# JeroendenBoef/GraphPOPE

Measured on AMD Instinct MI355X. Metric: POPE embeddings/sec (nodes x anchors) + SAGE nodes/sec, Flickr 256 anchors, higher is better.
Workload: dtype u64; 1 GPU; configs[1]: flickr-shaped geodesic-stochastic, N=89250 E=899756 F=500, 256 anchors PER GPU (np.random seed 42); inputs resident in HBM (edge_index, x) -> [N, F+K] f32 in HBM on every rank; anchors_total=256, anchors_per_rank=256, parallelism=single GPU

## Files before the change

### graphpope_amd/csrc/geodesic_level.h

```cpp
#pragma once

#ifdef POPE_STAMP
__device__ unsigned long long g_stamps[16384 * 8];
__device__ int g_stamp_level;
#define STAMP(slot)                                                                         \
    do {                                                                                    \
        __builtin_amdgcn_sched_barrier(0);                                                  \
        if (lane == 0 && wave < 16384 && level == g_stamp_level) g_stamps[wave * 8 + (slot)] = __builtin_amdgcn_s_memrealtime(); \
        __builtin_amdgcn_sched_barrier(0);                                                  \
    } while (0)
#else
#define STAMP(slot) do { } while (0)
#endif

template <int WT> struct Words { u64 w[WT]; };

typedef float f32x4 __attribute__((ext_vector_type(4)));

constexpr int DPP_ROW_SHR1 = 0x111, DPP_ROW_SHR2 = 0x112, DPP_ROW_SHR4 = 0x114, DPP_ROW_SHR8 = 0x118, DPP_ROW_BCAST15 = 0x142,
              DPP_ROW_BCAST31 = 0x143, DPP_WAVE_SHL1 = 0x130, DPP_WAVE_SHR1 = 0x138;
template <int CTRL>
__device__ __forceinline__ int dpp_mov(int x) { return __builtin_amdgcn_update_dpp(0, x, CTRL, 0xf, 0xf, true); }
template <int CTRL>
__device__ __forceinline__ u64 dpp_mov64(u64 x) {
    const unsigned lo = (unsigned)dpp_mov<CTRL>((int)(unsigned)x), hi = (unsigned)dpp_mov<CTRL>((int)(unsigned)(x >> 32));
    return ((u64)hi << 32) | lo;
}

template <int WT>
__device__ __forceinline__ Words<WT> load_words(const u64 *__restrict__ p) {
    Words<WT> r;
    if constexpr (WT == 1) {
        r.w[0] = p[0];
    } else {
#pragma unroll
        for (int i = 0; i < WT; i += 2) {
            const ulonglong2 v = *reinterpret_cast<const ulonglong2 *>(p + i);
            r.w[i] = v.x;
            r.w[i + 1] = v.y;
        }
    }
    return r;
}

typedef unsigned long long u64x2v __attribute__((ext_vector_type(2)));
typedef int i32x4v __attribute__((ext_vector_type(4)));
template <int WT, bool NT>
__device__ __forceinline__ Words<WT> load_words_hint(const u64 *__restrict__ p) {
    if constexpr (!NT) return load_words<WT>(p);
    Words<WT> r;
    if constexpr (WT == 1) {
        r.w[0] = __builtin_nontemporal_load(p);
    } else {
#pragma unroll
        for (int i = 0; i < WT; i += 2) {
            const u64x2v v = __builtin_nontemporal_load(reinterpret_cast<const u64x2v *>(p + i));
            r.w[i] = v.x;
            r.w[i + 1] = v.y;
        }
    }
    return r;
}

template <int WT>
__device__ __forceinline__ Words<WT> gather_words(const u64 *__restrict__ p) { return load_words<WT>(p); }

template <int WT>
__device__ __forceinline__ void store_words(u64 *__restrict__ p, const Words<WT> &r) {
    if constexpr (WT == 1) {
        p[0] = r.w[0];
    } else {
#pragma unroll
        for (int i = 0; i < WT; i += 2) *reinterpret_cast<ulonglong2 *>(p + i) = make_ulonglong2(r.w[i], r.w[i + 1]);
    }
}

template <int WT, bool NT>
__device__ __forceinline__ void store_words_hint(u64 *__restrict__ p, const Words<WT> &r) {
    if constexpr (!NT) {
        store_words<WT>(p, r);
    } else if constexpr (WT == 1) {
        __builtin_nontemporal_store(r.w[0], p);
    } else {
#pragma unroll
        for (int i = 0; i < WT; i += 2) {
            const u64x2v v = {r.w[i], r.w[i + 1]};
            __builtin_nontemporal_store(v, reinterpret_cast<u64x2v *>(p + i));
        }
    }
}

template <int WT>
__device__ __forceinline__ u64 any_bits(const Words<WT> &r) {
    u64 a = 0;
#pragma unroll
    for (int i = 0; i < WT; ++i) a |= r.w[i];
    return a;
}

template <int WT, bool NT = false>
__device__ __forceinline__ void commit_words(const Words<WT> &fresh, const Words<WT> &seen_old, size_t idx,
                                             u64 *__restrict__ seen, u64 *__restrict__ hop_planes,
                                             size_t plane_elems, int level) {
    Words<WT> s;
#pragma unroll
    for (int i = 0; i < WT; ++i) s.w[i] = seen_old.w[i] | fresh.w[i];
    store_words_hint<WT, NT>(seen + idx, s);
    Words<WT> h[5];
#pragma unroll
    for (int b = 0; b < 5; ++b) {
        h[b] = fresh;
        if ((level >> b) & 1) h[b] = load_words_hint<WT, NT>(hop_planes + (size_t)b * plane_elems + idx);
    }
#pragma unroll
    for (int b = 0; b < 5; ++b)
        if ((level >> b) & 1) {
#pragma unroll
            for (int i = 0; i < WT; ++i) h[b].w[i] |= fresh.w[i];
            store_words_hint<WT, NT>(hop_planes + (size_t)b * plane_elems + idx, h[b]);
        }
    for (int b = 5, l = level >> 5; l; ++b, l >>= 1)
        if (l & 1) {
            u64 *p = hop_planes + (size_t)b * plane_elems + idx;
            Words<WT> g = load_words_hint<WT, NT>(p);
#pragma unroll
            for (int i = 0; i < WT; ++i) g.w[i] |= fresh.w[i];
            store_words_hint<WT, NT>(p, g);
        }
}

__device__ __forceinline__ void stage_live_table(const unsigned *__restrict__ live, int live_words, uint4 *live_lds4) {
    const uint4 *src = reinterpret_cast<const uint4 *>(live);
    const int n4 = (live_words + 3) / 4;
    for (int base = 0; base < n4; base += 4 * 256) {
        uint4 t[4];
        int idx[4];
#pragma unroll
        for (int j = 0; j < 4; ++j) idx[j] = min(base + (int)threadIdx.x + 256 * j, n4 - 1);
#pragma unroll
        for (int j = 0; j < 4; ++j) t[j] = src[idx[j]];
#pragma unroll
        for (int j = 0; j < 4; ++j) live_lds4[idx[j]] = t[j];
    }
}

__global__ __launch_bounds__(256) void k_live_summary(const unsigned *__restrict__ live, int padded_words, unsigned *__restrict__ sum) {
    const int w = blockIdx.x * blockDim.x + threadIdx.x;
    const unsigned v = w < padded_words ? live[w] : 0u;
    const unsigned long long b = __ballot(v != 0u);
    if ((threadIdx.x & 63) == 0 && w < padded_words) {
        sum[(w >> 5)] = (unsigned)b;
        sum[(w >> 5) + 1] = (unsigned)(b >> 32);
    }
}

template <int WT, int LIVE, int TILES>
__device__ __forceinline__ void level_housekeeping(int E, int N, int Wp, int tiles_arg, const u64 *__restrict__ front, u64 *__restrict__ seen,
                                                   u64 *__restrict__ idle, u64 *__restrict__ hop_planes, size_t plane_elems, int level,
                                                   const int *aux, const unsigned *__restrict__ live, unsigned *__restrict__ live_idle,
                                                   int live_words, int t0, int tstride) {
    const int tiles = TILES ? tiles_arg : 1;
    const int n = (E + CHUNK - 1) >> CHUNK_SHIFT;
    const int *mrows = aux + AUX_HEADER;
    for (int i = t0; i < live_words; i += tstride) live_idle[i] = 0u;
    Words<WT> zero;
#pragma unroll
    for (int i = 0; i < WT; ++i) zero.w[i] = 0;
    for (int i = t0; i < n; i += tstride) {
        const int mv = mrows[i];
        if (mv >= 0)
            for (int t = 0; t < tiles; ++t) store_words<WT>(idle + (size_t)mv * Wp + t * WT, zero);
    }
    if (level > 1) {
        for (int v = t0; v < N; v += tstride) {
            if (!((live[v >> 5] >> (v & 31)) & 1u)) continue;
            constexpr bool NT = LIVE >= 2 && POPE_NT_PLANES != 0;
            for (int t = 0; t < tiles; ++t) {
                const size_t idx = (size_t)v * Wp + t * WT;
                const Words<WT> fresh = load_words<WT>(front + idx);
                if (any_bits<WT>(fresh))
                    commit_words<WT, NT>(fresh, load_words_hint<WT, NT>(seen + idx), idx, seen, hop_planes, plane_elems, level - 1);
            }
        }
    }
}

__device__ __forceinline__ int2 chunk_edge_rows(const int *__restrict__ erow, int chunk, int E) {
    int2 r = make_int2(-1, -2);
    if (chunk > 0 && chunk * CHUNK - 1 < E) r.x = erow[chunk * CHUNK - 1];
    if ((chunk + 1) * CHUNK < E) r.y = erow[(chunk + 1) * CHUNK];
    return r;
}

template <int WT, int LIVE, int TILES>
__device__ __forceinline__ bool level_expand(const int *__restrict__ erow, const int *__restrict__ col, int E, int Wp, int tile_begin, int tile_end,
                                             const u64 *__restrict__ front, u64 *__restrict__ seen, u64 *__restrict__ acc,
                                             const unsigned *__restrict__ live, unsigned *__restrict__ live_acc,
                                             const unsigned *live_lds, int level, int lane, int wave, int nwaves, int nchunks,
                                             int4 vr, int4 ur, unsigned *wave_words) {
    auto load_idx = [&](const int *p) {
        if constexpr (LIVE >= 2 && POPE_NT_INDEX != 0) {
            const i32x4v t = __builtin_nontemporal_load(reinterpret_cast<const i32x4v *>(p));
            return make_int4(t.x, t.y, t.z, t.w);
        } else {
            return *reinterpret_cast<const int4 *>(p);
        }
    };
    constexpr bool LOOP = TILES == 1;
    constexpr int TILE_AHEAD = LOOP ? (WT == 8 ? POPE_WT8_PREFETCH : POPE_TILE_PREFETCH) : 0;
    if (!TILES) { tile_begin = 0; tile_end = 1; }
    bool found = false;
    STAMP(0);
    auto live4 = [&](int u0, int u1, int u2, int u3, bool &q0, bool &q1, bool &q2, bool &q3) {
        if constexpr (LIVE == 3) {
            const bool s0 = (live_lds[u0 >> 10] >> ((u0 >> 5) & 31)) & 1u, s1 = (live_lds[u1 >> 10] >> ((u1 >> 5) & 31)) & 1u,
                       s2 = (live_lds[u2 >> 10] >> ((u2 >> 5) & 31)) & 1u, s3 = (live_lds[u3 >> 10] >> ((u3 >> 5) & 31)) & 1u;
            const unsigned w0 = live[s0 ? u0 >> 5 : 0], w1 = live[s1 ? u1 >> 5 : 0], w2 = live[s2 ? u2 >> 5 : 0], w3 = live[s3 ? u3 >> 5 : 0];
            q0 = s0 & ((w0 >> (u0 & 31)) & 1u); q1 = s1 & ((w1 >> (u1 & 31)) & 1u);
            q2 = s2 & ((w2 >> (u2 & 31)) & 1u); q3 = s3 & ((w3 >> (u3 & 31)) & 1u);
        } else {
            const unsigned *t = LIVE == 1 ? live_lds : live;
            const unsigned w0 = t[u0 >> 5], w1 = t[u1 >> 5], w2 = t[u2 >> 5], w3 = t[u3 >> 5];
            q0 = (w0 >> (u0 & 31)) & 1u; q1 = (w1 >> (u1 & 31)) & 1u; q2 = (w2 >> (u2 & 31)) & 1u; q3 = (w3 >> (u3 & 31)) & 1u;
        }
    };
    constexpr bool AHEAD = (LIVE >= 2 || (WT == 8 && POPE_L2_LOOP != 0)) && POPE_AHEAD != 0;
    constexpr bool AHEAD_LIVE = AHEAD && POPE_AHEAD == 1;
    auto slots_of = [&](int chunk, const int4 &vr_, const int4 &ur_, int &v0, int &v1, int &v2, int &v3, int &u0, int &u1, int &u2, int &u3) {
        const int base = chunk * CHUNK + lane * SLOTS;
        v0 = v1 = v2 = v3 = -1;
        u0 = u1 = u2 = u3 = 0;
        if (base < E) {
            v0 = vr_.x; u0 = ur_.x;
            if (base + 1 < E) { v1 = vr_.y; u1 = ur_.y; }
            if (base + 2 < E) { v2 = vr_.z; u2 = ur_.z; }
            if (base + 3 < E) { v3 = vr_.w; u3 = ur_.w; }
        }
    };
    bool q0 = false, q1 = false, q2 = false, q3 = false;
    if (AHEAD_LIVE && wave < nchunks) {
        int a0, a1, a2, a3, b0, b1, b2, b3;
        slots_of(wave, vr, ur, a0, a1, a2, a3, b0, b1, b2, b3);
        live4(b0, b1, b2, b3, q0, q1, q2, q3);
    }
    for (int chunk = wave; chunk < nchunks; chunk += nwaves) {
        STAMP(7);
        if (!AHEAD && chunk != wave && chunk * CHUNK + lane * SLOTS < E) {
            vr = load_idx(erow + chunk * CHUNK + lane * SLOTS);
            ur = load_idx(col + chunk * CHUNK + lane * SLOTS);
        }
        int v0, v1, v2, v3, u0, u1, u2, u3;
        slots_of(chunk, vr, ur, v0, v1, v2, v3, u0, u1, u2, u3);
        int4 vr_n = make_int4(-1, -1, -1, -1), ur_n = make_int4(0, 0, 0, 0);
        bool qn0 = false, qn1 = false, qn2 = false, qn3 = false;
        const int chunk_n = chunk + nwaves;
        if (AHEAD && chunk_n < nchunks && chunk_n * CHUNK + lane * SLOTS < E) {
            vr_n = load_idx(erow + chunk_n * CHUNK + lane * SLOTS);
            ur_n = load_idx(col + chunk_n * CHUNK + lane * SLOTS);
        }
        auto next_live = [&]() {
            if constexpr (AHEAD_LIVE) {
                if (chunk_n < nchunks) {
                    int a0, a1, a2, a3, b0, b1, b2, b3;
                    slots_of(chunk_n, vr_n, ur_n, a0, a1, a2, a3, b0, b1, b2, b3);
                    live4(b0, b1, b2, b3, qn0, qn1, qn2, qn3);
                }
            }
        };
        auto advance = [&]() {
            if constexpr (AHEAD) { vr = vr_n; ur = ur_n; }
            if constexpr (AHEAD_LIVE) { q0 = qn0; q1 = qn1; q2 = qn2; q3 = qn3; }
        };
        if constexpr (!AHEAD_LIVE) live4(u0, u1, u2, u3, q0, q1, q2, q3);
        const bool g0 = (v0 >= 0) & q0, g1 = (v1 >= 0) & q1, g2 = (v2 >= 0) & q2, g3 = (v3 >= 0) & q3;
        const int vc = __builtin_amdgcn_readlane(v0, 0);
        const int vl = __builtin_amdgcn_readlane(v3, 63);
        STAMP(1);
        const bool work = __any(g0 || g1 || g2 || g3);
        if (!work) {
            next_live();
            advance();
            continue;
        }
        const int2 er = chunk_edge_rows(erow, __builtin_amdgcn_readfirstlane(chunk), E);
        const bool head_multi = chunk > 0 && er.x == vc;
        const bool tail_multi = vl >= 0 && (chunk + 1) * CHUNK < E && er.y == vl;
        const bool x0 = (head_multi && v0 == vc) || (tail_multi && v0 == vl);
        const bool x1 = (head_multi && v1 == vc) || (tail_multi && v1 == vl);
        const bool x2 = (head_multi && v2 == vc) || (tail_multi && v2 == vl);
        const bool x3 = (head_multi && v3 == vc) || (tail_multi && v3 == vl);
        const int nv0 = dpp_mov<DPP_WAVE_SHL1>(v0);
        const int after3 = lane == 63 ? -3 : nv0;
        const bool e0 = v0 >= 0 && v0 != v1, e1 = v1 >= 0 && v1 != v2, e2 = v2 >= 0 && v2 != v3, e3 = v3 >= 0 && v3 != after3;
        const int pv3 = dpp_mov<DPP_WAVE_SHR1>(v3);
        const bool connects = lane > 0 && pv3 == v0 && v0 >= 0;
        const bool head0 = !(connects && v0 == v3);
        bool lv0, lv1, lv2, lv3;
        live4(max(v0, 0), max(v1, 0), max(v2, 0), max(v3, 0), lv0, lv1, lv2, lv3);
        bool m0 = false, m1 = false, m2 = false, m3 = false;
        const bool dense = TILES != 0;

        auto gather4 = [&](int woff, Words<WT> &c0, Words<WT> &c1, Words<WT> &c2, Words<WT> &c3) {
#pragma unroll
            for (int i = 0; i < WT; ++i) c0.w[i] = c1.w[i] = c2.w[i] = c3.w[i] = 0;
            if (g0) c0 = gather_words<WT>(front + (size_t)u0 * Wp + woff);
            if (g1) c1 = gather_words<WT>(front + (size_t)u1 * Wp + woff);
            if (g2) c2 = gather_words<WT>(front + (size_t)u2 * Wp + woff);
            if (g3) c3 = gather_words<WT>(front + (size_t)u3 * Wp + woff);
        };
        Words<WT> c0, c1, c2, c3, d0, d1, d2, d3;
        gather4(tile_begin * WT, c0, c1, c2, c3);
        if (TILE_AHEAD == 2 && tile_begin + 1 < tile_end) gather4((tile_begin + 1) * WT, d0, d1, d2, d3);
        next_live();
        for (int tile = tile_begin; tile < tile_end; ++tile) {
            const int woff = tile * WT;
            {
                auto row_mask = [&](int v, bool lv) {
                    Words<WT> m = load_words_hint<WT, LIVE >= 2 && POPE_NT_PLANES != 0>(seen + (size_t)v * Wp + woff);
                    if (lv) {
                        const Words<WT> f = load_words<WT>(front + (size_t)v * Wp + woff);
#pragma unroll
                        for (int i = 0; i < WT; ++i) m.w[i] |= f.w[i];
                    }
                    return m;
                };
                Words<WT> s0, s1, s2, s3;
#pragma unroll
                for (int i = 0; i < WT; ++i) s0.w[i] = s1.w[i] = s2.w[i] = s3.w[i] = 0;
                if (v0 >= 0) s0 = row_mask(v0, lv0);
                if (v3 >= 0) s3 = v3 == v0 ? s0 : row_mask(v3, lv3);
                if (v1 >= 0) s1 = v1 == v0 ? s0 : (v1 == v3 ? s3 : row_mask(v1, lv1));
                if (v2 >= 0) s2 = v2 == v1 ? s1 : (v2 == v3 ? s3 : row_mask(v2, lv2));
#pragma unroll
                for (int i = 0; i < WT; ++i) {
                    c0.w[i] &= ~s0.w[i];
                    c1.w[i] &= ~s1.w[i];
                    c2.w[i] &= ~s2.w[i];
                    c3.w[i] &= ~s3.w[i];
                }
            }
            if (TILE_AHEAD == 1 && tile + 1 < tile_end) gather4(woff + WT, d0, d1, d2, d3);
            const u64 any = any_bits<WT>(c0) | any_bits<WT>(c1) | any_bits<WT>(c2) | any_bits<WT>(c3);
            if (tile == tile_begin) STAMP(2);
            if (__any(any != 0)) {
#pragma unroll
                for (int i = 0; i < WT; ++i) {
                    if (v1 == v0) c1.w[i] |= c0.w[i];
                    if (v2 == v1) c2.w[i] |= c1.w[i];
                    if (v3 == v2) c3.w[i] |= c2.w[i];
                }
                Words<WT> t = c3;
                bool head = head0;
                auto scan_step = [&](auto ctrl, bool valid) {
                    constexpr int CTRL = decltype(ctrl)::value;
                    if (!__any(valid && !head)) return;
                    const bool ph = dpp_mov<CTRL>((int)head) != 0;
                    const bool take = valid && !head;
#pragma unroll
                    for (int i = 0; i < WT; ++i) {
                        const u64 pt = dpp_mov64<CTRL>(t.w[i]);
                        if (take) t.w[i] |= pt;
                    }
                    if (take) head = ph;
                };
                const int in_row = lane & 15;
                scan_step(std::integral_constant<int, DPP_ROW_SHR1>{}, in_row >= 1);
                scan_step(std::integral_constant<int, DPP_ROW_SHR2>{}, in_row >= 2);
                scan_step(std::integral_constant<int, DPP_ROW_SHR4>{}, in_row >= 4);
                scan_step(std::integral_constant<int, DPP_ROW_SHR8>{}, in_row >= 8);
                scan_step(std::integral_constant<int, DPP_ROW_BCAST15>{}, ((lane >> 4) & 1) != 0);
                scan_step(std::integral_constant<int, DPP_ROW_BCAST31>{}, lane >= 32);
#pragma unroll
                for (int i = 0; i < WT; ++i) {
                    u64 ci = dpp_mov64<DPP_WAVE_SHR1>(t.w[i]);
                    if (!connects) ci = 0;
                    c0.w[i] |= ci;
                    if (v1 == v0) c1.w[i] |= ci;
                    if (v2 == v0) c2.w[i] |= ci;
                    if (v3 == v0) c3.w[i] |= ci;
                }
            }
            if (tile == tile_begin) STAMP(3);
            const size_t i0 = (size_t)v0 * Wp + woff, i1 = (size_t)v1 * Wp + woff, i2 = (size_t)v2 * Wp + woff,
                         i3 = (size_t)v3 * Wp + woff;
            const bool n0 = e0 && any_bits<WT>(c0) != 0, n1 = e1 && any_bits<WT>(c1) != 0, n2 = e2 && any_bits<WT>(c2) != 0,
                       n3 = e3 && any_bits<WT>(c3) != 0;
            if (e0 && !x0 && (n0 || dense)) store_words<WT>(acc + i0, c0);
            if (e1 && !x1 && (n1 || dense)) store_words<WT>(acc + i1, c1);
            if (e2 && !x2 && (n2 || dense)) store_words<WT>(acc + i2, c2);
            if (e3 && !x3 && (n3 || dense)) store_words<WT>(acc + i3, c3);
            if (head_multi || tail_multi) {
                auto piece = [&](size_t idx, const Words<WT> &c) {
#pragma unroll
                    for (int i = 0; i < WT; ++i) atomicOr(&acc[idx + i], c.w[i]);
                };
                if (n0 && x0) piece(i0, c0);
                if (n1 && x1) piece(i1, c1);
                if (n2 && x2) piece(i2, c2);
                if (n3 && x3) piece(i3, c3);
            }
            if (tile == tile_begin) STAMP(4);
            m0 |= n0; m1 |= n1; m2 |= n2; m3 |= n3;
            if (TILE_AHEAD == 1 && tile + 1 < tile_end) { c0 = d0; c1 = d1; c2 = d2; c3 = d3; }
            else if (TILE_AHEAD == 2 && tile + 1 < tile_end) {
                if (!((tile - tile_begin) & 1)) { c0 = d0; c1 = d1; c2 = d2; c3 = d3; }
                else {
                    gather4(woff + WT, c0, c1, c2, c3);
                    if (tile + 2 < tile_end) gather4(woff + 2 * WT, d0, d1, d2, d3);
                }
            } else if (LOOP && tile + 1 < tile_end) gather4(woff + WT, c0, c1, c2, c3);
        }
        found |= m0 || m1 || m2 || m3;
        if (__any(m0 || m1 || m2 || m3)) {
            const int wfirst = vc >> 5;
            const int last_row = vl >= 0 ? vl : erow[min((chunk + 1) * CHUNK, E) - 1];
            const int kmax = (last_row >> 5) - wfirst;
            if (kmax < 8) {
                if (lane < 8) wave_words[lane] = 0u;
                if (m0) atomicOr(&wave_words[(v0 >> 5) - wfirst], 1u << (v0 & 31));
                if (m1) atomicOr(&wave_words[(v1 >> 5) - wfirst], 1u << (v1 & 31));
                if (m2) atomicOr(&wave_words[(v2 >> 5) - wfirst], 1u << (v2 & 31));
                if (m3) atomicOr(&wave_words[(v3 >> 5) - wfirst], 1u << (v3 & 31));
                __builtin_amdgcn_wave_barrier();
                if (lane <= kmax) {
                    const unsigned m = wave_words[lane];
                    if (m) atomicOr(&live_acc[wfirst + lane], m);
                }
            } else {
                if (m0) atomicOr(&live_acc[v0 >> 5], 1u << (v0 & 31));
                if (m1) atomicOr(&live_acc[v1 >> 5], 1u << (v1 & 31));
                if (m2) atomicOr(&live_acc[v2 >> 5], 1u << (v2 & 31));
                if (m3) atomicOr(&live_acc[v3 >> 5], 1u << (v3 & 31));
            }
        }
        STAMP(5);
        advance();
    }
    STAMP(6);
    return found;
}

template <int WT, int LIVE, int TILES>
__global__ __launch_bounds__(256, WT == 8 ? (TILES == 1 ? POPE_WT8_LOOP_WAVES : (LIVE == 1 ? POPE_WT8_L2_WAVES : POPE_WT8_WAVES)) : 1) void k_bfs_level(const int *__restrict__ erow, const int *__restrict__ col,
                                                   int E, int N, int Wp, int tiles, const u64 *__restrict__ front,
                                                   u64 *__restrict__ seen, u64 *__restrict__ acc,
                                                   u64 *__restrict__ idle, u64 *__restrict__ hop_planes,
                                                   size_t plane_elems, int level, BfsCtl *ctl, const int *aux,
                                                   int expand_blocks, const unsigned *__restrict__ live,
                                                   unsigned *__restrict__ live_acc, unsigned *__restrict__ live_idle,
                                                   int live_words, const unsigned *__restrict__ live_sum, int sum_words) {
    if (bfs_over(ctl, aux, level)) return;
    const int lane = threadIdx.x & 63;
    if ((int)blockIdx.x >= expand_blocks) {
        const int hb = (int)gridDim.x - expand_blocks;
        level_housekeeping<WT, LIVE, TILES>(E, N, Wp, tiles, front, seen, idle, hop_planes, plane_elems, level, aux, live, live_idle, live_words,
                                     ((int)blockIdx.x - expand_blocks) * blockDim.x + threadIdx.x, hb * blockDim.x);
        return;
    }
    int wave = (blockIdx.x * blockDim.x + threadIdx.x) >> 6, nwaves = (expand_blocks * blockDim.x) >> 6, tile_begin = 0, tile_end = tiles;
    if constexpr (TILES == 2) {
        const int wid = wave;
        wave = wid / tiles;
        tile_begin = wid - wave * tiles;
        tile_end = tile_begin + 1;
        nwaves /= tiles;
    }
    const int nchunks = (E + CHUNK - 1) >> CHUNK_SHIFT;
    int4 vr = make_int4(-1, -1, -1, -1), ur = make_int4(0, 0, 0, 0);
    if (wave < nchunks && wave * CHUNK + lane * SLOTS < E) {
        if constexpr (LIVE >= 2 && POPE_NT_INDEX != 0) {
            const i32x4v a = __builtin_nontemporal_load(reinterpret_cast<const i32x4v *>(erow + wave * CHUNK + lane * SLOTS));
            const i32x4v b = __builtin_nontemporal_load(reinterpret_cast<const i32x4v *>(col + wave * CHUNK + lane * SLOTS));
            vr = make_int4(a.x, a.y, a.z, a.w);
            ur = make_int4(b.x, b.y, b.z, b.w);
        } else {
            vr = *reinterpret_cast<const int4 *>(erow + wave * CHUNK + lane * SLOTS);
            ur = *reinterpret_cast<const int4 *>(col + wave * CHUNK + lane * SLOTS);
        }
    }
    extern __shared__ uint4 live_lds4[];
    const unsigned *live_lds = reinterpret_cast<const unsigned *>(live_lds4);
    if constexpr (LIVE == 1) {
        stage_live_table(live, live_words, live_lds4);
        __syncthreads();
    } else if constexpr (LIVE == 3) {
        stage_live_table(live_sum, sum_words, live_lds4);
        __syncthreads();
    }
    __shared__ unsigned wave_live_words[4][8];
    const bool found = level_expand<WT, LIVE, TILES>(erow, col, E, Wp, tile_begin, tile_end, front, seen, acc, live, live_acc, live_lds, level, lane, wave, nwaves,
                                              nchunks, vr, ur, wave_live_words[threadIdx.x >> 6]);
    if (__any(found) && lane == 0) raise_level(ctl, level);
}
```

Baseline: 100.2 billion embeddings/s.

## Apply seen/front masks after segmented scan using per-lane distinct row loads

For non-WT8, non-single-tile variants, the visited/frontier mask is no longer computed per tile for all four edge slots before the scan. Each lane identifies at most two distinct destination rows (first and last ending segment) plus optional middle rows, and issues their seen/front loads up front, before the gather, so they overlap it. The mask is applied after the scan, and the middle-row loads run only when some lane needs them. This cuts redundant mask loads and moves their latency off the critical path, at the cost of more branching and more live registers. The stamp buffer is also resized to 16 slots per wave for the new probe point.

```diff
diff --git a/graphpope_amd/csrc/geodesic_level.h b/graphpope_amd/csrc/geodesic_level.h
--- a/graphpope_amd/csrc/geodesic_level.h
+++ b/graphpope_amd/csrc/geodesic_level.h
@@ -1,12 +1,12 @@
 #pragma once
 
 #ifdef POPE_STAMP
-__device__ unsigned long long g_stamps[16384 * 8];
+__device__ unsigned long long g_stamps[8192 * 16];
 __device__ int g_stamp_level;
 #define STAMP(slot)                                                                         \
     do {                                                                                    \
         __builtin_amdgcn_sched_barrier(0);                                                  \
-        if (lane == 0 && wave < 16384 && level == g_stamp_level) g_stamps[wave * 8 + (slot)] = __builtin_amdgcn_s_memrealtime(); \
+        if (lane == 0 && wave < 8192 && level == g_stamp_level) g_stamps[wave * 16 + (slot)] = __builtin_amdgcn_s_memrealtime(); \
         __builtin_amdgcn_sched_barrier(0);                                                  \
     } while (0)
 #else
@@ -295,8 +295,16 @@
         const int pv3 = dpp_mov<DPP_WAVE_SHR1>(v3);
         const bool connects = lane > 0 && pv3 == v0 && v0 >= 0;
         const bool head0 = !(connects && v0 == v3);
-        bool lv0, lv1, lv2, lv3;
-        live4(max(v0, 0), max(v1, 0), max(v2, 0), max(v3, 0), lv0, lv1, lv2, lv3);
+        constexpr bool EMIT_MASK = WT != 8 && TILES != 1;
+        const bool mid1 = e1 && e0 && (e2 || e3), mid2 = e2 && e3 && (e0 || e1);
+        const bool any_mid = EMIT_MASK && __any(mid1 || mid2);
+        const int vP = e0 ? v0 : e1 ? v1 : e2 ? v2 : e3 ? v3 : vc;
+        const int vS = e3 ? v3 : e2 ? v2 : e1 ? v1 : e0 ? v0 : vc;
+        const int vM1 = mid1 ? v1 : vc, vM2 = mid2 ? v2 : vc;
+        bool lvP = false, lvS = false, lvM1 = false, lvM2 = false;
+        bool lv0 = false, lv1 = false, lv2 = false, lv3 = false;
+        if constexpr (EMIT_MASK) live4(vP, vS, vM1, vM2, lvP, lvS, lvM1, lvM2);
+        else live4(max(v0, 0), max(v1, 0), max(v2, 0), max(v3, 0), lv0, lv1, lv2, lv3);
         bool m0 = false, m1 = false, m2 = false, m3 = false;
         const bool dense = TILES != 0;
 
@@ -308,15 +316,30 @@
             if (g2) c2 = gather_words<WT>(front + (size_t)u2 * Wp + woff);
             if (g3) c3 = gather_words<WT>(front + (size_t)u3 * Wp + woff);
         };
+        constexpr bool NT_MASK = LIVE >= 2 && POPE_NT_PLANES != 0;
+        auto mask_request = [&](int woff, int va, bool la, int vb, bool lb, Words<WT> &sa, Words<WT> &fa, Words<WT> &sb, Words<WT> &fb) {
+            sa = load_words_hint<WT, NT_MASK>(seen + (size_t)va * Wp + woff);
+            fa = load_words<WT>(front + (size_t)(la ? va : vc) * Wp + woff);
+            sb = load_words_hint<WT, NT_MASK>(seen + (size_t)vb * Wp + woff);
+            fb = load_words<WT>(front + (size_t)(lb ? vb : vc) * Wp + woff);
+        };
+        auto mask_of = [&](const Words<WT> &s, const Words<WT> &f, bool l) {
+            Words<WT> m;
+#pragma unroll
+            for (int i = 0; i < WT; ++i) m.w[i] = s.w[i] | (l ? f.w[i] : 0);
+            return m;
+        };
+        Words<WT> ps, pf, ss, sf;
+        if constexpr (EMIT_MASK) mask_request(tile_begin * WT, vP, lvP, vS, lvS, ps, pf, ss, sf);
         Words<WT> c0, c1, c2, c3, d0, d1, d2, d3;
         gather4(tile_begin * WT, c0, c1, c2, c3);
         if (TILE_AHEAD == 2 && tile_begin + 1 < tile_end) gather4((tile_begin + 1) * WT, d0, d1, d2, d3);
         next_live();
         for (int tile = tile_begin; tile < tile_end; ++tile) {
             const int woff = tile * WT;
-            {
+            if constexpr (!EMIT_MASK) {
                 auto row_mask = [&](int v, bool lv) {
-                    Words<WT> m = load_words_hint<WT, LIVE >= 2 && POPE_NT_PLANES != 0>(seen + (size_t)v * Wp + woff);
+                    Words<WT> m = load_words_hint<WT, NT_MASK>(seen + (size_t)v * Wp + woff);
                     if (lv) {
                         const Words<WT> f = load_words<WT>(front + (size_t)v * Wp + woff);
 #pragma unroll
@@ -381,6 +404,33 @@
                 }
             }
             if (tile == tile_begin) STAMP(3);
+            if constexpr (EMIT_MASK) {
+                const Words<WT> mP = mask_of(ps, pf, lvP), mS = mask_of(ss, sf, lvS);
+                Words<WT> k1, k2;
+#pragma unroll
+                for (int i = 0; i < WT; ++i) {
+                    k1.w[i] = e0 ? mS.w[i] : mP.w[i];
+                    k2.w[i] = e3 ? mP.w[i] : mS.w[i];
+                }
+                if (any_mid) {
+                    Words<WT> s1, f1, s2, f2;
+                    mask_request(woff, vM1, lvM1, vM2, lvM2, s1, f1, s2, f2);
+                    const Words<WT> mM1 = mask_of(s1, f1, lvM1), mM2 = mask_of(s2, f2, lvM2);
+#pragma unroll
+                    for (int i = 0; i < WT; ++i) {
+                        if (mid1) k1.w[i] = mM1.w[i];
+                        if (mid2) k2.w[i] = mM2.w[i];
+                    }
+                }
+#pragma unroll
+                for (int i = 0; i < WT; ++i) {
+                    c0.w[i] &= ~mP.w[i];
+                    c1.w[i] &= ~k1.w[i];
+                    c2.w[i] &= ~k2.w[i];
+                    c3.w[i] &= ~mS.w[i];
+                }
+            }
+            if (tile == tile_begin) STAMP(8);
             const size_t i0 = (size_t)v0 * Wp + woff, i1 = (size_t)v1 * Wp + woff, i2 = (size_t)v2 * Wp + woff,
                          i3 = (size_t)v3 * Wp + woff;
             const bool n0 = e0 && any_bits<WT>(c0) != 0, n1 = e1 && any_bits<WT>(c1) != 0, n2 = e2 && any_bits<WT>(c2) != 0,
```

Result: slower. 95.66 billion embeddings/s (-4.5%).
